# RustAudio/rodio

Measured on AMD Instinct MI355X. Metric: Msamples/s through resample+low_pass+mix pipeline, higher is better.
Workload: dtype f32; 1 GPU; 256 f32 stereo sources/GPU x 1048576 frames, 44.1->48 kHz linear resample + low_pass(200) + ordered Mixer sum, span_len=None; numpy default_rng(1234+s) U(-1,1)/256; in_frames=1048576, out_frames=1141308, channels=2, kernel=k_rlm_chunk

## Files before the change

rodio_amd/csrc/rh_pipeline.hip:

```cpp
#include "rh_pipeline_dev.h"

namespace {


__device__ __forceinline__ uint32_t rag_find_pairs(const Params &p, const uint32_t m_tile0, const uint32_t m_stable, const int lane, lds_u8 *lds, const uint32_t list_off);
template <int R, int KV, int C>
__device__ __forceinline__ void rag_run_pairs(const Params &p, unsigned long long *const rows, const uint32_t tile, const uint32_t n_pairs, const int lane, lds_u8 *lds, const uint32_t lds0,
                                              const uint32_t list_off, const uint32_t i_base, const uint32_t nvec, const uint32_t (&goff)[KV], const int (&offA)[R + 2], const float (&wgt)[R + 2],
                                              const float (&lM)[4], const float (&b15)[4], const float (&b31)[4], const float (&kM)[4], typename Chan<C>::V (&acc)[R]);

template <int R, int KV, int NS, bool FILT, bool RAG = false, int C = 2, bool SUMF = false>
__global__ __launch_bounds__(64, (R <= 4 ? (KV <= 5 ? 5 : 4) : R <= 6 ? 3 : R <= 12 ? 2 : 1)) void k_rlm_fast(const Params p) {
    typedef Chan<C> CH;
    typedef typename CH::V V;
    constexpr uint32_t FB = CH::kFB, VF = CH::kVF;
    static_assert(R <= kMaxR, "frames per lane");
    static_assert(NS >= 2 && NS <= 4, "ring depth");
    static_assert(KV * (NS - 1) < 64, "vmcnt range");
    constexpr uint32_t kStage = KV * 1024;
    extern __shared__ __attribute__((aligned(16))) unsigned char smem[];
    lds_u8 *const lds = (lds_u8 *)smem;
    const uint32_t lds0 = (uint32_t)(uintptr_t)lds;

    const int lane = threadIdx.x;
// ... 1124 lines not shown
            for (int u = 0; u < U; ++u) {
                const v4f v = __builtin_nontemporal_load(ptr + base + (uint64_t)u * 256u);
                acc[u].x = fma_(g, v.x, acc[u].x);
                acc[u].y = fma_(g, v.y, acc[u].y);
                acc[u].z = fma_(g, v.z, acc[u].z);
                acc[u].w = fma_(g, v.w, acc[u].w);
            }
        }
#pragma unroll
        for (int u = 0; u < U; ++u) *reinterpret_cast<v4f *>(y + 4 * (base + (uint64_t)u * 256u)) = acc[u];
    } else {
        for (int u = 0; u < U; ++u) {
            const uint64_t i = base + (uint64_t)u * 256u;
            if (i >= nvec) break;
            v4f a = v4f{0.f, 0.f, 0.f, 0.f};
            for (uint32_t s = 0; s < n_sources; ++s) {
                glb_cf4 *const ptr = (glb_cf4 *)(uintptr_t)(desc[4 * (uint64_t)s] + src_off);
                const float g = dgain[8 * (uint64_t)s + 4];
                const v4f v = ptr[i];
                a.x = fma_(g, v.x, a.x), a.y = fma_(g, v.y, a.y), a.z = fma_(g, v.z, a.z), a.w = fma_(g, v.w, a.w);
            }
            *reinterpret_cast<v4f *>(y + 4 * i) = a;
        }
    }
    if (blockIdx.x == 0) {
        const uint64_t t = nvec * 4 + threadIdx.x;
        if (t < n_floats) {
            float a = 0.f;
            for (uint32_t s = 0; s < n_sources; ++s) a = fma_(dgain[8 * (uint64_t)s + 4], ((glb_cf32 *)(uintptr_t)(desc[4 * (uint64_t)s] + src_off))[t], a);
            y[t] = a;
        }
        if (threadIdx.x == 0) {
            ydesc->data = desc_row;
            ydesc->frames = frames;
            ydesc->out_frames = out_frames;
            ydesc->gain = 1.0f;
            ydesc->pad[0] = ydesc->pad[1] = ydesc->pad[2] = 0;
        }
    }
}

template <int NS>
__global__ __launch_bounds__(64) void k_mix_ring(const SrcDesc *__restrict__ srcs, const uint32_t n_sources, float *__restrict__ y, const uint64_t n_floats, SrcDesc *__restrict__ ydesc,
                                                 const uint32_t frames, const uint32_t out_frames, const float *desc_row, const uint64_t src_off) {
    constexpr int KV = 8;
    constexpr uint32_t kStage = KV * 1024;
    __shared__ __attribute__((aligned(1024))) unsigned char smem[NS * kStage];
    lds_u8 *const lds = (lds_u8 *)smem;
    const uint32_t lds0 = (uint32_t)(uintptr_t)lds;
    typedef __attribute__((address_space(4))) const uint64_t cu64;
    typedef __attribute__((address_space(4))) const float cf32;
    cu64 *const desc = (cu64 *)(uintptr_t)srcs;
    cf32 *const dgain = (cf32 *)(uintptr_t)srcs;
    const int lane = threadIdx.x;
    const uint64_t nvec = n_floats / 4;
    const uint64_t v0 = (uint64_t)blockIdx.x * (KV * 64);
    uint32_t goff[KV];
#pragma unroll
    for (int k = 0; k < KV; ++k) {
        uint64_t j = v0 + (uint64_t)k * 64 + lane;
        j = j < nvec ? j : nvec - 1;
        goff[k] = (uint32_t)(j * 16);
    }
    auto stage_source = [&](uint32_t s_, uint32_t stage) {
        const void *data = (const void *)(uintptr_t)(desc[4 * (uint64_t)s_] + src_off);
#pragma unroll
        for (int k = 0; k < KV; ++k) glds16(data, goff[k], lds0 + stage * kStage + k * 1024);
    };
    v4f acc[KV];
#pragma unroll
    for (int k = 0; k < KV; ++k) acc[k] = v4f{0.f, 0.f, 0.f, 0.f};
    if (v0 < nvec) {
#pragma unroll
        for (int d = 0; d < NS - 1; ++d)
            if ((uint32_t)d < n_sources) stage_source(d, d);
        uint32_t st = 0;
        float g_next = n_sources ? dgain[4] : 0.f;
        for (uint32_t s_ = 0; s_ < n_sources; ++s_) {
            const float g = g_next;
            g_next = s_ + 1 < n_sources ? dgain[8 * (uint64_t)(s_ + 1) + 4] : 0.f;
            if (s_ + NS - 1 < n_sources) {
                uint32_t into = st + NS - 1;
                into = into >= (uint32_t)NS ? into - NS : into;
                stage_source(s_ + NS - 1, into);
                wait_vm<KV *(NS - 1)>();
            } else {
                const uint32_t left = n_sources - 1 - s_;
                wait_groups<KV, NS>((int)left);
            }
            const lds_u8 *buf = lds + st * kStage;
            v4f v[KV];
#pragma unroll
            for (int k = 0; k < KV; ++k) v[k] = *(const lds_f4 *)(buf + k * 1024 + lane * 16);
            asm volatile("s_waitcnt lgkmcnt(0)" ::: "memory");
#pragma unroll
            for (int k = 0; k < KV; ++k) {
                acc[k].x = fma_(g, v[k].x, acc[k].x);
                acc[k].y = fma_(g, v[k].y, acc[k].y);
                acc[k].z = fma_(g, v[k].z, acc[k].z);
                acc[k].w = fma_(g, v[k].w, acc[k].w);
            }
            st = st + 1 == (uint32_t)NS ? 0 : st + 1;
        }
        wait_vm<0>();
#pragma unroll
        for (int k = 0; k < KV; ++k) {
            const uint64_t j = v0 + (uint64_t)k * 64 + lane;
            if (j < nvec) *reinterpret_cast<v4f *>(y + 4 * j) = acc[k];
        }
    }
    if (blockIdx.x == 0) {
        const uint64_t t = nvec * 4 + lane;
        if (t < n_floats) {
            float a = 0.f;
            for (uint32_t s_ = 0; s_ < n_sources; ++s_) a = fma_(dgain[8 * (uint64_t)s_ + 4], ((glb_cf32 *)(uintptr_t)(desc[4 * (uint64_t)s_] + src_off))[t], a);
            y[t] = a;
        }
        if (lane == 0) {
            ydesc->data = desc_row;
            ydesc->frames = frames;
            ydesc->out_frames = out_frames;
            ydesc->gain = 1.0f;
            ydesc->pad[0] = ydesc->pad[1] = ydesc->pad[2] = 0;
        }
    }
}

struct ChunkArgs {
    const uint32_t *m_lo;
    unsigned long long *halo;
    const float *lookT;
    const float *powM;
    const float *uni;
};
constexpr uint32_t kChunkMultiMax = 7;
struct ChunkMulti {
    struct Entry {
        Params p;
        ChunkArgs q;
    };
    uint32_t n;
    uint32_t first[kChunkMultiMax + 1];
    float *sum_out;
    Entry e[kChunkMultiMax];
};
static_assert(sizeof(ChunkMulti) <= 4096, "the kernarg segment");
#if defined(RH_CHUNK_DIAG) && RH_CHUNK_DIAG == 3
#define RH_CPH(i) { const unsigned long long cph_now = __builtin_readcyclecounter(); if (lane == 0) atomicAdd(p.ticket + 8 + (i), (uint32_t)(cph_now - cph_last)); cph_last = cph_now; }
#define RH_CPH_DECL unsigned long long cph_last = __builtin_readcyclecounter();
#else
#define RH_CPH(i)
#define RH_CPH_DECL
#endif
template <int R, int C, int KV>
__device__ __forceinline__ void rlm_chunk_tile(const Params &p, const ChunkArgs &q, const uint32_t block) {
    typedef Chan<C> CH;
    typedef typename CH::V V;
    constexpr int NS = 2, H = 4;
    constexpr uint32_t FB = CH::kFB;
    constexpr uint32_t kStage = KV * 1024, P = kStage / FB;
    constexpr uint32_t MB = NS * kStage + 64;
    __shared__ __attribute__((aligned(1024))) unsigned char smem[MB + kStage + 64];
    lds_u8 *const lds = (lds_u8 *)smem;
    const uint32_t lds0 = (uint32_t)(uintptr_t)lds;
    typedef __attribute__((address_space(4))) const uint64_t cu64;
    typedef __attribute__((address_space(4))) const float cf32;
    typedef __attribute__((address_space(4))) const uint32_t cu32;
    cu64 *const desc = (cu64 *)(uintptr_t)p.srcs;
    cf32 *const dgain = (cf32 *)(uintptr_t)p.srcs;
    const int lane = threadIdx.x;
    uint32_t tile = block;
    if (!p.direct) {
        const uint32_t x = block & 7u;
        const uint32_t k = __builtin_amdgcn_readfirstlane(lane == 0 ? atomicAdd(p.ticket + 32u * (1u + x), 1u) - p.shard_base : 0u);
        tile = x + 8u * k;
        if (tile >= p.n_tiles) return;
    }
#ifdef RH_CHUNK_RAGSIM
    const uint32_t Ns = p.eq_frames;
    const uint32_t S = 2u * tile < p.n_tiles ? p.n_sources : (uint32_t)(((uint64_t)p.n_sources * 2u * (p.n_tiles - tile)) / p.n_tiles);
#else
    const uint32_t Ns = p.eq_frames, S = p.n_sources;
#endif
    const uint32_t m_lo = ((cu32 *)(uintptr_t)q.m_lo)[tile], m_hi = ((cu32 *)(uintptr_t)q.m_lo)[tile + 1];
    const uint32_t m0 = m_lo + (uint32_t)lane * R;
    int nfl;
    uint32_t n_t_v;
    float pwv[4];
    {
        const uint32_t n_t = m_hi - m_lo;
        nfl = (int)n_t - lane * R < 0 ? 0 : ((int)n_t - lane * R > R ? R : (int)n_t - lane * R);
        const uint32_t nl0 = (n_t + R - 1) / R;
        const uint32_t v = nl0 ? n_t - (nl0 - 1) * R : 0;
        n_t_v = n_t;
        asm volatile("v_mov_b32 %0, %1" : "=v"(n_t_v) : "s"(n_t));
        const float *pw = q.powM + 4 * v;
#pragma unroll
        for (int k = 0; k < 4; ++k) {
            pwv[k] = pw[k];
            asm volatile("" : "+v"(pwv[k]));
        }
    }
    const bool first = (m0 == 0);

    const uint32_t nvec = Ns * C / 4;
    const uint32_t v0 = tile * (KV * 64);
    uint32_t goff[KV];
#pragma unroll
    for (int k = 0; k < KV; ++k) {
        uint32_t j = v0 + (uint32_t)k * 64 + lane;
        j = j < nvec ? j : nvec - 1;
        goff[k] = j * 16;
    }
    const bool lin = v0 + (uint32_t)(KV * 64) <= nvec;
    auto stage_source = [&](uint32_t s_, uint32_t stage) {
        const void *data = (const void *)(uintptr_t)desc[4 * (uint64_t)s_];
        if (lin) {
            glds16_run<KV>(data, goff[0], lds0 + stage * kStage);
        } else {
#pragma unroll
            for (int k = 0; k < KV; ++k) glds16(data, goff[k], lds0 + stage * kStage + k * 1024);
        }
    };
    if (S) stage_source(0, 0);
    if (S > 1) stage_source(1, 1);
    const Tables *__restrict__ tb = p.tabs;
    float lM[4], b15[4], b31[4], kM[4];
    constexpr int NHV = H * FB / 16;
    const uint32_t Jc = p.J < tile ? p.J : tile;
    int want_look = (uint32_t)lane < Jc ? 1 : 0;
    uint64_t a_halo_pub = (uint64_t)(uintptr_t)(q.halo + (uint64_t)tile * 8 + (uint32_t)(lane >= 64 - NHV ? lane - (64 - NHV) : 0) * 4);
    uint64_t a_halo_poll = (uint64_t)(uintptr_t)(q.halo + (uint64_t)(tile ? tile - 1 : 0) * 8 + (lane < H * C ? lane : 0));
    uint64_t a_gran_pub = (uint64_t)(uintptr_t)(p.gran + (uint64_t)tile * 4 + (lane < 2 * C ? lane : 0));
    uint64_t a_gran_poll = (uint64_t)(uintptr_t)(p.gran + (uint64_t)(tile ? tile - 1 - (want_look ? lane : 0) : 0) * 4);
    uint64_t a_out = (uint64_t)(uintptr_t)(p.out + ((uint64_t)m_lo + (uint32_t)lane) * C);
    uint32_t epoch_v = p.epoch;
    float U = q.uni[lane < 61 ? lane : 60];
    asm volatile("" : "+v"(want_look), "+v"(a_halo_pub), "+v"(a_halo_poll), "+v"(a_gran_pub), "+v"(a_gran_poll), "+v"(a_out), "+v"(epoch_v), "+v"(U));
    {
        const uint32_t Jc0 = Jc;
        const float *kp = q.lookT + ((uint64_t)tile * p.J + ((uint32_t)lane < Jc0 ? lane : 0)) * 4;
#pragma unroll
        for (int k = 0; k < 4; ++k) {
            lM[k] = tb->laneM[lane][k];
            b15[k] = tb->bc15M[lane][k];
            b31[k] = tb->bc31M[lane][k];
            kM[k] = kp[k];
        }
    }
    int offA[R + 2];
    float wgt[R + 2];
    {
        const int64_t fbase = (int64_t)tile * P;
        Cursor c = cursor_at(first ? 0 : m0 - 2, p);
#pragma unroll
        for (int rr = 0; rr < R + 2; ++rr) {
#if defined(RH_CHUNK_DIAG) && RH_CHUNK_DIAG == 2
            offA[rr] = (int)MB + rr * 8;
            wgt[rr] = 0.5f;
            continue;
#endif
            const bool dummy = first && rr < 2;
            uint64_t i;
            uint32_t num;
            cursor_resolve(c, p, i, num);
            if (i + 1 >= Ns) {
                i = Ns - 1;
                num = 0;
            }
            int64_t f = (int64_t)i - fbase;
            f = f < -H ? -H : (f > (int64_t)P - 1 ? (int64_t)P - 1 : f);
            offA[rr] = dummy ? (int)MB : (int)MB + (int)f * (int)FB;
            wgt[rr] = dummy ? 0.0f : (float)num / p.Tf;
            if (!dummy) cursor_next(c, p);
        }
    }
    v4f acc[KV];
#pragma unroll
    for (int k = 0; k < KV; ++k) acc[k] = v4f{0.f, 0.f, 0.f, 0.f};
    {
        uint32_t st = 0;
        float g_next = S ? dgain[4] : 0.f;
        for (uint32_t s_ = 0; s_ < S; ++s_) {
            const float g = g_next;
            g_next = s_ + 1 < S ? dgain[8 * (uint64_t)(s_ + 1) + 4] : 0.f;
            if (s_ + 1 < S) wait_vm<KV>();
            else wait_vm<0>();
            const lds_u8 *buf = lds + st * kStage;
            v4f v[KV];
#pragma unroll
            for (int k = 0; k < KV; ++k) v[k] = *(const lds_f4 *)(buf + k * 1024 + lane * 16);
            asm volatile("s_waitcnt lgkmcnt(0)" ::: "memory");
            if (s_ + 2 < S) stage_source(s_ + 2, st);
#pragma unroll
            for (int k = 0; k < KV; ++k) {
                acc[k].x = fma_(g, v[k].x, acc[k].x);
                acc[k].y = fma_(g, v[k].y, acc[k].y);
                acc[k].z = fma_(g, v[k].z, acc[k].z);
                acc[k].w = fma_(g, v[k].w, acc[k].w);
            }
            st ^= 1u;
        }
    }
    RH_CPH_DECL
#if defined(RH_CHUNK_DIAG) && RH_CHUNK_DIAG < 3
    {
        float t = 0.f;
#pragma unroll
        for (int k = 0; k < KV; ++k) t += acc[k].x + acc[k].y + acc[k].z + acc[k].w;
#pragma unroll
        for (int rr = 0; rr < R + 2; ++rr) t += wgt[rr] + (float)offA[rr];
        p.out[(uint64_t)tile * 64 + lane] = t + lM[0] + b15[0] + b31[0] + kM[0] + (float)nfl + (first ? 1.f : 0.f);
        return;
    }
#endif
    if (lane >= 64 - NHV) {
        unsigned long long *hp = (unsigned long long *)(uintptr_t)a_halo_pub;
        const float e[4] = {acc[KV - 1].x, acc[KV - 1].y, acc[KV - 1].z, acc[KV - 1].w};
#pragma unroll
        for (int w = 0; w < 4; ++w) __hip_atomic_store(hp + w, ((unsigned long long)epoch_v << 32) | __float_as_uint(e[w]), __ATOMIC_RELAXED, __HIP_MEMORY_SCOPE_AGENT);
    }
#pragma unroll
    for (int k = 0; k < KV; ++k) *(lds_f4 *)(lds + MB + (uint32_t)(k * 64 + lane) * 16) = acc[k];
    if (lane == 0) *(lds_f4 *)(lds + MB + kStage) = v4f{0.f, 0.f, 0.f, 0.f};
    bool dead = false;
    if (tile == 0) {
        if (lane < H * C) *(RH_LDS float *)(lds + MB - H * FB + lane * 4) = 0.0f;
    } else {
        const bool want = lane < H * C;
        const unsigned long long *hp = (const unsigned long long *)(uintptr_t)a_halo_poll;
        unsigned long long hv = 0;
        bool ok = false;
        uint32_t spins = 0;
        while (true) {
            if (want && !ok) {
                hv = __hip_atomic_load(hp, __ATOMIC_RELAXED, __HIP_MEMORY_SCOPE_AGENT);
                ok = (uint32_t)(hv >> 32) == epoch_v;
            }
            if (__all(ok || !want)) break;
            if (++spins > kSpinLimit) {
                if (lane == 0) atomicOr(p.status, 1u);
                dead = true;
                break;
            }
            __builtin_amdgcn_s_sleep(1);
        }
        if (want) *(RH_LDS float *)(lds + MB - H * FB + lane * 4) = dead ? __builtin_nanf("") : __uint_as_float((uint32_t)hv);
    }
    asm volatile("s_waitcnt lgkmcnt(0)" ::: "memory");
    __builtin_amdgcn_wave_barrier();
    RH_CPH(0)

    const float b0 = readlane_f(U, 0), c1 = readlane_f(U, 1), c2 = readlane_f(U, 2), na1 = -readlane_f(U, 3), na2 = -readlane_f(U, 4);
    V out[R];
    V E1 = CH::zero(), E2 = CH::zero();
    {
        V ta[R + 2], tb2[R + 2];
#pragma unroll
        for (int rr = 0; rr < R + 2; ++rr) {
            ta[rr] = CH::ld_lds(lds + offA[rr]);
            tb2[rr] = CH::ld_lds(lds + offA[rr] + FB);
        }
        auto tap = [&](int rr) -> V {
            V x;
#pragma unroll
            for (int ch = 0; ch < C; ++ch) CH::set(x, ch, fma_(CH::get(tb2[rr], ch) - CH::get(ta[rr], ch), wgt[rr], CH::get(ta[rr], ch)));
            return x;
        };
        V x2 = first ? CH::zero() : tap(0);
        V x1 = first ? CH::zero() : tap(1);
        V w1 = CH::zero(), w2 = CH::zero();
#pragma unroll
        for (int r = 0; r < R; ++r) {
            const V x = tap(r + 2);
            V w;
#pragma unroll
            for (int ch = 0; ch < C; ++ch) {
                const float wc = fma_(na1, CH::get(w1, ch), fma_(na2, CH::get(w2, ch), fma_(c2, CH::get(x2, ch), c1 * CH::get(x1, ch))));
                CH::set(w, ch, wc);
                CH::set(out[r], ch, fma_(b0, CH::get(x, ch), wc));
            }
            w2 = w1;
            w1 = w;
            x2 = x1;
            x1 = x;
            E1 = vsel(r + 1 == nfl, w1, E1);
            E2 = vsel(r + 1 == nfl, w2, E2);
        }
    }
    RH_CPH(1)
    float Pq[2 * C];
#pragma unroll
    for (int k = 0; k < 2 * C; ++k) Pq[k] = 0.f;
    {
        const float Tm[4] = {readlane_f(U, 5), readlane_f(U, 6), readlane_f(U, 7), readlane_f(U, 8)};
#pragma unroll
        for (int ch = 0; ch < C; ++ch) mat_acc(Tm, CH::get(E1, ch), CH::get(E2, ch), Pq[2 * ch], Pq[2 * ch + 1]);
    }
    float own[2 * C];
#pragma unroll
    for (int k = 0; k < 2 * C; ++k) own[k] = Pq[k];
#define RH_CSCAN(K, N)                                                                             \
    {                                                                                              \
        float sq[2 * C];                                                                           \
        _Pragma("unroll") for (int k = 0; k < 2 * C; ++k) sq[k] = dpp0<kDppRowShr + N, 0xf>(Pq[k]); \
        const float sM[4] = {readlane_f(U, 9 + 4 * K), readlane_f(U, 10 + 4 * K), readlane_f(U, 11 + 4 * K), readlane_f(U, 12 + 4 * K)}; \
        _Pragma("unroll") for (int ch = 0; ch < C; ++ch) mat_acc(sM, sq[2 * ch], sq[2 * ch + 1], Pq[2 * ch], Pq[2 * ch + 1]); \
    }
    RH_CSCAN(0, 1)
    RH_CSCAN(1, 2)
    RH_CSCAN(2, 4)
    RH_CSCAN(3, 8)
#undef RH_CSCAN
    {
        float sq[2 * C];
#pragma unroll
        for (int k = 0; k < 2 * C; ++k) sq[k] = dpp0<kDppBcast15, 0xa>(Pq[k]);
#pragma unroll
        for (int ch = 0; ch < C; ++ch) mat_acc(b15, sq[2 * ch], sq[2 * ch + 1], Pq[2 * ch], Pq[2 * ch + 1]);
    }
    {
        float sq[2 * C];
#pragma unroll
        for (int k = 0; k < 2 * C; ++k) sq[k] = dpp0<kDppBcast31, 0xc>(Pq[k]);
#pragma unroll
        for (int ch = 0; ch < C; ++ch) mat_acc(b31, sq[2 * ch], sq[2 * ch + 1], Pq[2 * ch], Pq[2 * ch + 1]);
    }
    {
        const uint32_t n_t = (uint32_t)__builtin_amdgcn_readfirstlane((int)n_t_v);
        const int nl = (int)((n_t + R - 1) / R);
        float A[2 * C];
#pragma unroll
        for (int k = 0; k < 2 * C; ++k) A[k] = 0.f;
        if (nl >= 1) {
#pragma unroll
            for (int k = 0; k < 2 * C; ++k) A[k] = __int_as_float(__builtin_amdgcn_readlane(__float_as_int(own[k]), nl - 1));
        }
        if (nl >= 2) {
            const float M[4] = {readfirstlane_f(pwv[0]), readfirstlane_f(pwv[1]), readfirstlane_f(pwv[2]), readfirstlane_f(pwv[3])};
            float xp[2 * C];
#pragma unroll
            for (int k = 0; k < 2 * C; ++k) xp[k] = __int_as_float(__builtin_amdgcn_readlane(__float_as_int(Pq[k]), nl - 2));
#pragma unroll
            for (int ch = 0; ch < C; ++ch) mat_acc(M, xp[2 * ch], xp[2 * ch + 1], A[2 * ch], A[2 * ch + 1]);
        }
        if (lane < 2 * C) {
            float ev = A[0];
#pragma unroll
            for (int k = 1; k < 2 * C; ++k) ev = lane == k ? A[k] : ev;
            __hip_atomic_store((unsigned long long *)(uintptr_t)a_gran_pub, ((unsigned long long)epoch_v << 32) | __float_as_uint(ev), __ATOMIC_RELAXED, __HIP_MEMORY_SCOPE_AGENT);
        }
    }
    float Q[2 * C];
#pragma unroll
    for (int k = 0; k < 2 * C; ++k) Q[k] = dpp0<kDppWaveShr1, 0xf>(Pq[k]);
    RH_CPH(2)
    float c[2 * C];
#pragma unroll
    for (int k = 0; k < 2 * C; ++k) c[k] = 0.f;
    if (tile > 0) {
        const bool want = want_look != 0;
        const unsigned long long *gp = (const unsigned long long *)(uintptr_t)a_gran_poll;
        unsigned long long gv[2 * C];
#pragma unroll
        for (int k = 0; k < 2 * C; ++k) gv[k] = 0;
        bool ok = false;
        uint32_t spins = 0;
        while (true) {
            if (want && !ok) {
                bool all = true;
#pragma unroll
                for (int k = 0; k < 2 * C; ++k) {
                    gv[k] = __hip_atomic_load(gp + k, __ATOMIC_RELAXED, __HIP_MEMORY_SCOPE_AGENT);
                    all = all && ((uint32_t)(gv[k] >> 32) == epoch_v);
                }
                ok = all;
            }
            if (__all(ok || !want)) break;
            if (++spins > kSpinLimit) {
                if (lane == 0) atomicOr(p.status, 1u);
                dead = true;
                break;
            }
            __builtin_amdgcn_s_sleep(4);
        }
        if (lane == 0 && spins) atomicAdd(p.status + 1, spins);
        if (want && ok && !dead) {
#pragma unroll
            for (int ch = 0; ch < C; ++ch) mat_acc(kM, __uint_as_float((uint32_t)gv[2 * ch]), __uint_as_float((uint32_t)gv[2 * ch + 1]), c[2 * ch], c[2 * ch + 1]);
        }
#pragma unroll
        for (int k = 0; k < 2 * C; ++k) {
            c[k] += dpp0<kDppRowShr + 1, 0xf>(c[k]);
            c[k] += dpp0<kDppRowShr + 2, 0xf>(c[k]);
            c[k] += dpp0<kDppRowShr + 4, 0xf>(c[k]);
            c[k] += dpp0<kDppRowShr + 8, 0xf>(c[k]);
            c[k] = readlane_f(c[k], 15) + readlane_f(c[k], 31);
        }
    }
    if (dead) {
#pragma unroll
        for (int k = 0; k < 2 * C; ++k) c[k] = __builtin_nanf("");
    }
    RH_CPH(3)
#pragma unroll
    for (int ch = 0; ch < C; ++ch) mat_acc(lM, c[2 * ch], c[2 * ch + 1], Q[2 * ch], Q[2 * ch + 1]);
    constexpr uint32_t kRow = (R + 1) * FB;
    {
        lds_u8 *row = lds + (uint32_t)lane * kRow;
#pragma unroll
        for (int r = 0; r < R; ++r) {
            V y;
#pragma unroll
            for (int ch = 0; ch < C; ++ch) CH::set(y, ch, fma_(readlane_f(U, 25 + 2 * r), Q[2 * ch], fma_(readlane_f(U, 26 + 2 * r), Q[2 * ch + 1], CH::get(out[r], ch))));
            if (C == 2) *(lds_f2 *)(row + r * FB) = v2f{CH::get(y, 0), CH::get(y, C - 1)};
            else *(RH_LDS float *)(row + r * FB) = CH::get(y, 0);
        }
    }
    asm volatile("s_waitcnt lgkmcnt(0)" ::: "memory");
    __builtin_amdgcn_wave_barrier();
    {
        const uint32_t n_t = (uint32_t)__builtin_amdgcn_readfirstlane((int)n_t_v);
        float *ot = (float *)(uintptr_t)a_out;
        for (uint32_t f0 = 0; f0 < n_t; f0 += 64) {
            const uint32_t f = f0 + (uint32_t)lane;
            if (f < n_t) {
                const lds_u8 *src2 = lds + (f / R) * kRow + (f % R) * FB;
                if (C == 2) {
                    const v2f a = *(const lds_f2 *)src2;
                    *reinterpret_cast<float2 *>(ot + (uint64_t)f0 * 2) = make_float2(a.x, a.y);
                } else {
                    ot[f0] = *(const RH_LDS float *)src2;
                }
            }
        }
    }
    RH_CPH(4)
}
template <int R, int C, int KV>
__global__ __launch_bounds__(64, 2) void k_rlm_chunk(const Params p, const ChunkArgs q) {
    rlm_chunk_tile<R, C, KV>(p, q, blockIdx.x);
}
template <int R, int C, int KV>
__global__ __launch_bounds__(64, 2) void k_rlm_chunk_multi(const ChunkMulti m) {
    uint32_t k = 0;
#pragma unroll
    for (uint32_t i = 1; i < kChunkMultiMax; ++i) k += (i < m.n && blockIdx.x >= m.first[i]) ? 1u : 0u;
    uint32_t b0 = 0;
#pragma unroll
    for (uint32_t i = 1; i < kChunkMultiMax; ++i) b0 = (i == k) ? m.first[i] : b0;
    k = __builtin_amdgcn_readfirstlane(k);
    typedef const __attribute__((address_space(4))) unsigned char *cbytes;
    cbytes e = (cbytes)__builtin_amdgcn_kernarg_segment_ptr() + offsetof(ChunkMulti, e) + (size_t)k * sizeof(ChunkMulti::Entry);
    Params p;
    ChunkArgs q;
    typedef const __attribute__((address_space(4))) uint32_t *cwords;
    static_assert(sizeof(Params) % 4 == 0 && sizeof(ChunkArgs) % 4 == 0 && offsetof(ChunkMulti::Entry, q) % 4 == 0, "copied word by word");
    {
        cwords wp = (cwords)(e + offsetof(ChunkMulti::Entry, p)), wq = (cwords)(e + offsetof(ChunkMulti::Entry, q));
        uint32_t *dp = reinterpret_cast<uint32_t *>(&p), *dq = reinterpret_cast<uint32_t *>(&q);
#pragma unroll
        for (uint32_t i = 0; i < sizeof(Params) / 4; ++i) dp[i] = wp[i];
#pragma unroll
        for (uint32_t i = 0; i < sizeof(ChunkArgs) / 4; ++i) dq[i] = wq[i];
    }
    rlm_chunk_tile<R, C, KV>(p, q, blockIdx.x - b0);
}

#if defined(RH_CLS_DIAG) && RH_CLS_DIAG == 9
__device__ unsigned long long g_cls_stamp[2048 * 8 * 8];
#define RH_CLS_STAMP(i) { if (lane == 0 && tile < 2048 && k < 8) g_cls_stamp[((uint64_t)tile * 8 + k) * 8 + (i)] = wall_clock64(); }
#else
#define RH_CLS_STAMP(i)
#endif
#define RH_PARG(T, e, f) (*(const __attribute__((address_space(4))) T *)((e) + offsetof(ChunkMulti::Entry, p) + offsetof(Params, f)))
#define RH_QARG(T, e, f) (*(const __attribute__((address_space(4))) T *)((e) + offsetof(ChunkMulti::Entry, q) + offsetof(ChunkArgs, f)))
template <int R, int C, int KV>
__global__ __launch_bounds__(128, 2) void k_rlm_chunk_classes(const ChunkMulti m) {
    typedef Chan<C> CH;
    typedef typename CH::V V;
    constexpr int NS = 2, H = 4;
    constexpr uint32_t FB = CH::kFB;
    constexpr uint32_t kStage = KV * 1024, P = kStage / FB;
    constexpr uint32_t kCtl = NS * kStage;
    constexpr uint32_t kImg = kStage + 128;
    constexpr uint32_t MB0 = kCtl + 64 + 64;
    __shared__ __attribute__((aligned(1024))) unsigned char smem[kCtl + 64 + 2 * kImg];
    lds_u8 *const lds = (lds_u8 *)smem;
    const uint32_t lds0 = (uint32_t)(uintptr_t)lds;
    typedef __attribute__((address_space(4))) const uint64_t cu64;
    typedef __attribute__((address_space(4))) const float cf32;
    typedef __attribute__((address_space(4))) const uint32_t cu32;
    typedef const __attribute__((address_space(4))) unsigned char *cbytes;
    const cbytes kseg = (cbytes)__builtin_amdgcn_kernarg_segment_ptr();
    const int wave = __builtin_amdgcn_readfirstlane((int)(threadIdx.x >> 6));
    const int lane = (int)(threadIdx.x & 63u);
    const uint32_t n_cls = m.n;
    const Params &p0 = m.e[0].p;
    const uint32_t tile = blockIdx.x;
    const uint32_t Ns = p0.eq_frames;
    auto entry = [&](uint32_t k) -> cbytes { return kseg + offsetof(ChunkMulti, e) + (size_t)k * sizeof(ChunkMulti::Entry); };
    auto ctl_read = [&](uint32_t which) -> uint32_t {
        uint32_t v;
        asm volatile("ds_read_b32 %0, %1\n\ts_waitcnt lgkmcnt(0)" : "=v"(v) : "v"(lds0 + kCtl + which * 4) : "memory");
        return (uint32_t)__builtin_amdgcn_readfirstlane((int)v);
    };
    auto ctl_write = [&](uint32_t which, uint32_t v) {
        asm volatile("s_waitcnt lgkmcnt(0)" ::: "memory");
        if (lane == 0) *(RH_LDS uint32_t *)(lds + kCtl + which * 4) = v;
        asm volatile("s_waitcnt lgkmcnt(0)" ::: "memory");
    };
    if (wave == 0) {
        if (lane < 2) *(RH_LDS uint32_t *)(lds + kCtl + lane * 4) = 0u;
    }
    asm volatile("s_waitcnt lgkmcnt(0)\n\ts_barrier" ::: "memory");
    if (wave == 0) {
        const uint32_t nvec = Ns * C / 4;
        const uint32_t v0 = tile * (KV * 64);
        uint32_t goff[KV];
#pragma unroll
        for (int k = 0; k < KV; ++k) {
            uint32_t j = v0 + (uint32_t)k * 64 + lane;
            j = j < nvec ? j : nvec - 1;
            goff[k] = j * 16;
        }
        const bool lin = v0 + (uint32_t)(KV * 64) <= nvec;
        auto stage_source = [&](cu64 *desc, uint32_t s_, uint32_t stage) {
            const void *data = (const void *)(uintptr_t)desc[4 * (uint64_t)s_];
            if (lin) {
                glds16_run<KV>(data, goff[0], lds0 + stage * kStage);
            } else {
#pragma unroll
                for (int k = 0; k < KV; ++k) glds16(data, goff[k], lds0 + stage * kStage + k * 1024);
            }
        };
        constexpr int NHV = H * FB / 16;
        __builtin_amdgcn_s_setprio(3);
        uint32_t kc = 0, sc = 0;
        cu64 *ndesc = (cu64 *)(uintptr_t)RH_PARG(uint64_t, entry(0), srcs);
        uint32_t nS = RH_PARG(uint32_t, entry(0), n_sources);
        uint32_t nstage = 0;
        auto request_next = [&]() {
            if (kc >= n_cls) return false;
            stage_source(ndesc, sc, nstage);
            nstage ^= 1u;
            if (++sc == nS) {
                sc = 0;
                if (++kc < n_cls) {
                    ndesc = (cu64 *)(uintptr_t)RH_PARG(uint64_t, entry(kc), srcs);
                    nS = RH_PARG(uint32_t, entry(kc), n_sources);
                }
            }
            return true;
        };
        uint32_t ahead = 0;
        if (request_next()) ++ahead;
        if (request_next()) ++ahead;
        uint32_t st = 0;
        for (uint32_t k = 0; k < n_cls; ++k) {
            const cbytes e = entry(k);
            cf32 *const dgain = (cf32 *)(uintptr_t)RH_PARG(uint64_t, e, srcs);
            const uint32_t S = RH_PARG(uint32_t, e, n_sources);
            v4f acc[KV];
#pragma unroll
            for (int i = 0; i < KV; ++i) acc[i] = v4f{0.f, 0.f, 0.f, 0.f};
            float g_next = S ? dgain[4] : 0.f;
            for (uint32_t s_ = 0; s_ < S; ++s_) {
                const float g = g_next;
                g_next = s_ + 1 < S ? dgain[8 * (uint64_t)(s_ + 1) + 4] : 0.f;
                if (ahead > 1) wait_vm<KV>();
                else wait_vm<0>();
                --ahead;
                const lds_u8 *buf = lds + st * kStage;
                v4f v[KV];
#pragma unroll
                for (int i = 0; i < KV; ++i) v[i] = *(const lds_f4 *)(buf + i * 1024 + lane * 16);
                asm volatile("s_waitcnt lgkmcnt(0)" ::: "memory");
                if (request_next()) ++ahead;
#pragma unroll
                for (int i = 0; i < KV; ++i) {
                    acc[i].x = fma_(g, v[i].x, acc[i].x);
                    acc[i].y = fma_(g, v[i].y, acc[i].y);
                    acc[i].z = fma_(g, v[i].z, acc[i].z);
                    acc[i].w = fma_(g, v[i].w, acc[i].w);
                }
                st ^= 1u;
            }
            RH_CLS_STAMP(0)
            if (lane >= 64 - NHV) {
                unsigned long long *hp = (unsigned long long *)(uintptr_t)RH_QARG(uint64_t, e, halo) + (uint64_t)tile * 8 + (uint32_t)(lane - (64 - NHV)) * 4;
// ... 624 lines not shown

#define RH_FAST(r, kv, ns) Variant{r, kv, ns, &k_rlm_fast<r, kv, ns, true>, &k_rlm_fast<r, kv, ns, false>}
#define RH_WAVE(r, kv, ns) Variant{r, kv, ns, &k_rlm_wave<r, kv, ns, true>, &k_rlm_wave<r, kv, ns, false>}
const Variant kFast[] = {
#ifdef RH_DEV_VARIANTS
    RH_FAST(4, 2, 2), RH_FAST(4, 2, 3), RH_FAST(5, 3, 2), RH_FAST(6, 3, 2), RH_FAST(6, 3, 3), RH_FAST(8, 4, 2), RH_FAST(8, 4, 3), RH_FAST(9, 5, 2), RH_FAST(9, 5, 3), RH_FAST(12, 6, 3),
#else
    RH_FAST(3, 2, 2),   RH_FAST(3, 2, 3),   RH_FAST(3, 4, 2),  RH_FAST(3, 7, 2),
    RH_FAST(4, 2, 2),   RH_FAST(4, 2, 3),   RH_FAST(4, 3, 2),  RH_FAST(4, 3, 3),  RH_FAST(4, 5, 2),  RH_FAST(4, 9, 2),
    RH_FAST(5, 3, 2),   RH_FAST(5, 3, 3),   RH_FAST(5, 6, 2),
    RH_FAST(6, 3, 2),   RH_FAST(6, 3, 3),   RH_FAST(6, 4, 2),  RH_FAST(6, 4, 3),  RH_FAST(6, 7, 2),  RH_FAST(6, 14, 2),
    RH_FAST(7, 4, 2),   RH_FAST(7, 4, 3),   RH_FAST(7, 8, 2),
    RH_FAST(8, 4, 2),   RH_FAST(8, 4, 3),   RH_FAST(8, 4, 4),  RH_FAST(8, 5, 2),  RH_FAST(8, 5, 3),  RH_FAST(8, 9, 2),
    RH_FAST(9, 5, 2),   RH_FAST(9, 5, 3),   RH_FAST(9, 10, 2),
    RH_FAST(10, 5, 2),  RH_FAST(10, 5, 3),  RH_FAST(10, 6, 2), RH_FAST(10, 6, 3), RH_FAST(10, 11, 2),
    RH_FAST(12, 6, 2),  RH_FAST(12, 6, 3),  RH_FAST(12, 7, 2), RH_FAST(12, 7, 3), RH_FAST(12, 13, 2),
    RH_FAST(14, 7, 2),  RH_FAST(14, 8, 2),
    RH_FAST(16, 8, 2),  RH_FAST(16, 8, 3),  RH_FAST(16, 9, 2), RH_FAST(16, 9, 3),
    RH_FAST(18, 9, 2),  RH_FAST(18, 9, 3),  RH_FAST(18, 10, 2),
    RH_FAST(20, 10, 2), RH_FAST(20, 10, 3), RH_FAST(20, 11, 2),
#endif
};
const Variant kWave[] = {
    RH_WAVE(6, 3, 2), RH_WAVE(6, 4, 2), RH_WAVE(6, 7, 2), RH_WAVE(6, 14, 2), RH_WAVE(8, 4, 2), RH_WAVE(8, 4, 3), RH_WAVE(8, 5, 2), RH_WAVE(8, 9, 2),
    RH_WAVE(9, 5, 2), RH_WAVE(9, 5, 3), RH_WAVE(10, 5, 2), RH_WAVE(10, 5, 3), RH_WAVE(10, 6, 2), RH_WAVE(12, 6, 2), RH_WAVE(12, 6, 3), RH_WAVE(12, 7, 2),
};
#ifdef RH_RAG_NO_SUMF
#define RH_RAGN(r, kv, ns) Variant{r, kv, ns, &k_rlm_fast<r, kv, ns, true, true>, &k_rlm_resid<r, kv>}
#else
#define RH_RAGN(r, kv, ns) Variant{r, kv, ns, &k_rlm_fast<r, kv, ns, true, true, 2, true>, &k_rlm_resid<r, kv>}
#endif
#define RH_RAG(r, kv) RH_RAGN(r, kv, 2)
const Variant kRag[] = {
    RH_RAG(6, 3), RH_RAG(6, 4), RH_RAG(6, 7), RH_RAG(6, 14), RH_RAG(8, 4), RH_RAG(8, 5), RH_RAG(8, 9), RH_RAG(9, 5), RH_RAG(10, 5), RH_RAG(10, 6), RH_RAG(12, 6), RH_RAG(12, 7),
    RH_RAG(14, 7), RH_RAG(14, 8), RH_RAG(18, 9), RH_RAG(18, 10),
};
const Variant kRag1[] = {
#define RH_RAG1(r, kv) Variant{r, kv, 2, &k_rlm_fast<r, kv, 2, true, true, 1, true>, nullptr}
    RH_RAG1(6, 2), RH_RAG1(8, 2), RH_RAG1(8, 3), RH_RAG1(10, 3), RH_RAG1(12, 3), RH_RAG1(12, 4), RH_RAG1(16, 4), RH_RAG1(16, 5), RH_RAG1(18, 5),
#undef RH_RAG1
};
#define RH_FAST1(r, kv, ns) Variant{r, kv, ns, &k_rlm_fast<r, kv, ns, true, false, 1>, &k_rlm_fast<r, kv, ns, false, false, 1>}
#define RH_WAVE1(r, kv, ns) Variant{r, kv, ns, &k_rlm_wave<r, kv, ns, true, 1>, &k_rlm_wave<r, kv, ns, false, 1>}
const Variant kFast1[] = {
    RH_FAST1(4, 2, 2),  RH_FAST1(4, 3, 2),  RH_FAST1(4, 5, 2),  RH_FAST1(6, 2, 2),  RH_FAST1(6, 4, 2),  RH_FAST1(6, 7, 2),  RH_FAST1(8, 2, 2),   RH_FAST1(8, 3, 2),
    RH_FAST1(8, 5, 2),  RH_FAST1(8, 10, 2), RH_FAST1(9, 3, 2),  RH_FAST1(9, 5, 2),  RH_FAST1(10, 3, 2), RH_FAST1(10, 6, 2), RH_FAST1(12, 3, 2),  RH_FAST1(12, 4, 2),
    RH_FAST1(12, 7, 2), RH_FAST1(16, 4, 2), RH_FAST1(16, 5, 2), RH_FAST1(16, 9, 2), RH_FAST1(18, 5, 2), RH_FAST1(18, 5, 3), RH_FAST1(18, 10, 2), RH_FAST1(20, 5, 2),
    RH_FAST1(20, 6, 2), RH_FAST1(20, 11, 2),
};
const Variant kWave1[] = {
    RH_WAVE1(6, 2, 2), RH_WAVE1(6, 4, 2), RH_WAVE1(6, 7, 2), RH_WAVE1(8, 2, 2),  RH_WAVE1(8, 3, 2),  RH_WAVE1(8, 5, 2),  RH_WAVE1(8, 10, 2),
    RH_WAVE1(9, 3, 2), RH_WAVE1(9, 5, 2), RH_WAVE1(10, 3, 2), RH_WAVE1(10, 6, 2), RH_WAVE1(12, 3, 2), RH_WAVE1(12, 4, 2), RH_WAVE1(12, 7, 2),
};
#undef RH_FAST1
#undef RH_WAVE1
#undef RH_RAG
#undef RH_RAGN
#undef RH_FAST
#undef RH_WAVE
}

namespace rhp {

VariantTab variant_tab(TabKind kind, bool mono) {
    switch (kind) {
    case kTabFast: return mono ? tab_of(kFast1) : tab_of(kFast);
    case kTabWave: return mono ? tab_of(kWave1) : tab_of(kWave);
    default: return mono ? tab_of(kRag1) : tab_of(kRag);
    }
}

const void *chunk_kernel(int R, uint32_t channels, int KV) {
    if (channels == 2 && R == 9 && KV == 4) return reinterpret_cast<const void *>(&k_rlm_chunk<9, 2, 4>);
    if (channels == 2 && R == 18 && KV == 8) return reinterpret_cast<const void *>(&k_rlm_chunk<18, 2, 8>);
    if (channels == 2 && R == 18 && KV == 4) return reinterpret_cast<const void *>(&k_rlm_chunk<18, 2, 4>);
    if (channels == 1 && R == 18 && KV == 4) return reinterpret_cast<const void *>(&k_rlm_chunk<18, 1, 4>);
    if (channels == 1 && R == 18 && KV == 2) return reinterpret_cast<const void *>(&k_rlm_chunk<18, 1, 2>);
    return nullptr;
}

static const void *chunk_multi_kernel(int R, uint32_t channels, int KV) {
    if (channels == 2 && R == 9 && KV == 4) return reinterpret_cast<const void *>(&k_rlm_chunk_multi<9, 2, 4>);
    if (channels == 2 && R == 18 && KV == 8) return reinterpret_cast<const void *>(&k_rlm_chunk_multi<18, 2, 8>);
    if (channels == 2 && R == 18 && KV == 4) return reinterpret_cast<const void *>(&k_rlm_chunk_multi<18, 2, 4>);
    if (channels == 1 && R == 18 && KV == 4) return reinterpret_cast<const void *>(&k_rlm_chunk_multi<18, 1, 4>);
    if (channels == 1 && R == 18 && KV == 2) return reinterpret_cast<const void *>(&k_rlm_chunk_multi<18, 1, 2>);
    return nullptr;
}

static const void *chunk_classes_kernel(int R, uint32_t channels, int KV) {
    if (channels == 2 && R == 18 && KV == 8) return reinterpret_cast<const void *>(&k_rlm_chunk_classes<18, 2, 8>);
    if (channels == 2 && R == 18 && KV == 4) return reinterpret_cast<const void *>(&k_rlm_chunk_classes<18, 2, 4>);
    if (channels == 1 && R == 18 && KV == 4) return reinterpret_cast<const void *>(&k_rlm_chunk_classes<18, 1, 4>);
    if (channels == 1 && R == 18 && KV == 2) return reinterpret_cast<const void *>(&k_rlm_chunk_classes<18, 1, 2>);
    return nullptr;
}

rh_status chunk_launch_classes(rh_rlm *const *classes, float *const *rows, uint64_t row_capacity_frames, uint32_t n, float *dst_sum, rh_stream stream, bool *taken, bool *summed) {
    *taken = false;
    *summed = false;
    if (n < 2 || n > kChunkMultiMax || rh::knob(rh::K_CLASSES_ONE_BY_ONE)) return RH_OK;
    const void *fn = nullptr;
    for (uint32_t k = 0; k < n; ++k) {
        const rh_rlm *h = classes[k];
        if (!h || !h->cls.empty() || !h->plan || h->out_frames == 0 || row_capacity_frames < h->out_frames) return RH_OK;
        if (!h->chunk.ok || !mix_first_applies(h, *h->plan, h->n_sources, false, false)) return RH_OK;
        const void *f = chunk_multi_kernel(h->chunk.R, h->cfg.channels, h->chunk.KV);
        if (!f || (fn && f != fn)) return RH_OK;
        fn = f;
    }
    ChunkMulti m;
    memset(&m, 0, sizeof m);
    for (uint32_t k = 0; k < n; ++k) {
        rh_rlm *h = classes[k];
        h->collect = &m;
        const rh_status st = rlm_launch(h, 0, h->n_sources, rows[k], row_capacity_frames, nullptr, stream, 0, 0, StreamArgs{});
        h->collect = nullptr;
        if (st != RH_OK) return st;
        if (m.n != k + 1) return RH_ERR_UNSUPPORTED;
    }
    void *args[] = {&m};
    hipStream_t s = rh::as_stream(stream);
    const void *fn2 = rh::knob(rh::K_CLASSES_ONE_WAVE) ? nullptr : chunk_classes_kernel(classes[0]->chunk.R, classes[0]->cfg.channels, classes[0]->chunk.KV);
    bool same = fn2 != nullptr;
    for (uint32_t k = 0; k < n && same; ++k) {
        const rh_rlm *h = classes[k], *h0 = classes[0];
        same = h->exclusive && h->eq_frames == h0->eq_frames && h->out_frames == h0->out_frames && h->F == h0->F && h->T == h0->T && h->chunk_in == h0->chunk_in &&
               h->chunk_out == h0->chunk_out && h->chunk.n_tiles == h0->chunk.n_tiles && h->chunk.R == h0->chunk.R && h->chunk.KV == h0->chunk.KV && h->n_sources >= 1;
    }
    if (same) {
        int per_cu = 0;
        same = hipOccupancyMaxActiveBlocksPerMultiprocessor(&per_cu, fn2, 128, 0) == hipSuccess && per_cu >= 1 &&
               (uint64_t)classes[0]->chunk.n_tiles <= (uint64_t)per_cu * (uint64_t)rh::g_num_cus;
    }
    hipError_t e;
    if (same) {
        m.sum_out = dst_sum;
        e = hipLaunchKernel(fn2, dim3(classes[0]->chunk.n_tiles), dim3(128), args, 0, s);
        *summed = e == hipSuccess;
    } else {
        e = hipLaunchKernel(fn, dim3(m.first[m.n]), dim3(64), args, 0, s);
        if (e == hipSuccess)
            for (uint32_t k = 0; k < n; ++k) classes[k]->shard_base += (m.first[k + 1] - m.first[k]) / 8u;
    }
    if (e != hipSuccess) {
        rh::set_hip_error(e, "k_rlm_chunk_multi / k_rlm_chunk_classes launch");
        return RH_ERR_HIP;
    }
    for (uint32_t k = 0; k < n; ++k) mark_launch(classes[k], s);
    *taken = true;
    return RH_OK;
}

#if defined(RH_CLS_DIAG) && RH_CLS_DIAG == 9
extern "C" int rh_debug_cls_stamps(unsigned long long *dst, size_t n) {
    return (int)hipMemcpyFromSymbol(dst, HIP_SYMBOL(g_cls_stamp), n * sizeof(unsigned long long), 0, hipMemcpyDeviceToHost);
}
#endif
void launch_state(hipStream_t s, unsigned long long *gran, const Tables *tabs, uint32_t n_sources, uint32_t cols, uint32_t last_col, uint32_t J, uint32_t epoch, uint32_t next_epoch) {
    hipLaunchKernelGGL(k_rlm_state, dim3((n_sources + 63) / 64), dim3(64), 0, s, gran, tabs, n_sources, cols, last_col, J, epoch, next_epoch);
}

void launch_state_sum(hipStream_t s, const unsigned long long *gran, const SrcDesc *srcs, uint32_t n_sources, uint32_t cols, uint32_t tag, float *w_out) {
    hipLaunchKernelGGL(k_rlm_state_sum, dim3(1), dim3(256), 0, s, gran, srcs, n_sources, cols, tag, w_out);
}

bool mix_first_applies(const rh_rlm *p, const Plan &pl, uint32_t count, bool per_source_states, bool batch) {
    return &pl == &p->fast && p->filt && p->mix_first_on && !per_source_states && !batch && count >= 2 && !rh::knob(rh::K_NO_MIX_FIRST);
}

rh_status rlm_launch(rh_rlm *p, uint32_t first, uint32_t count, float *dst, uint64_t out_capacity_frames, uint64_t *out_frames, rh_stream stream, uint32_t batch_streams, uint64_t out_stride,
                            const StreamArgs &sa) {
    RH_REQUIRE_INIT();
    if (!p) return RH_ERR_INVALID;
    if (!p->cls.empty()) return RH_ERR_UNSUPPORTED;
    if (first > p->n_sources || count > p->n_sources - first) return RH_ERR_INVALID;
    if (out_frames) *out_frames = p->out_frames;
    if (p->out_frames == 0) return RH_OK;
    if (!dst || (reinterpret_cast<uintptr_t>(dst) & 15u)) return RH_ERR_INVALID;
    if (out_capacity_frames < p->out_frames) return RH_ERR_CAPACITY;
    hipStream_t s = rh::as_stream(stream);
    {
        const rh_status w = pre_launch(p, s);
        if (w != RH_OK) return w;
    }
    const Plan &pl = *p->plan;
    {
        const rh_status w = next_epoch(p, s);
        if (w != RH_OK) return w;
    }
    Params k;
    k.srcs = p->d_srcs + first;
    k.tabs = pl.d_tabs;
    k.out = dst;
    k.gran = p->d_gran;
    k.ticket = p->d_ctl;
    k.status = p->d_ctl + 1;
    k.out_frames = p->out_frames;
    k.chunk_in = sa.mode ? p->st_chunk_in : p->chunk_in;
    k.chunk_out = sa.mode ? p->st_chunk_out : p->chunk_out;
    k.n_sources = count;
    k.n_tiles = p->n_tiles;
    k.F = p->F;
    k.T = p->T;
    k.qF = p->F / p->T;
    k.rF = p->F % p->T;
    k.Tf = (float)p->T;
    k.rcpT = rh::lerp_rcp(p->T);
    k.epoch = p->epoch;
    k.J = pl.J;
    k.ticket_base = p->ticket_base;
    k.direct = 0;
    k.rag_merge = k.rag_pairs_from = k.rag_pairs_to = 0;
    k.prof = p->d_prof;
    k.eq_frames = p->eq_frames;
    k.batch_streams = batch_streams;
    k.shards = (batch_streams >= 16 && batch_streams % 8 == 0 && !rh::knob(rh::K_NO_TICKET_SHARDS)) ? 8u : 1u;
    k.shard_base = p->shard_base;
    k.out_stride = out_stride;
    k.st_mode = sa.mode;
    k.st_active = sa.active;
    k.st_m0 = sa.m0;
    k.st_g0 = sa.g0;
    k.st_mfirst = sa.mode ? p->st_mfirst : 0;
    k.st_win = sa.win;
    k.st_wout = sa.wout;
    k.gran_cols = sa.gran_cols ? sa.gran_cols : p->n_tiles;
    k.col0 = sa.gran_cols ? 1u : 0u;
    k.u = pl.uni;
    void *args[] = {&k};
    const uint64_t grid = (uint64_t)p->n_tiles * (batch_streams ? batch_streams : 1);
    if (grid > 0x7fffffffull) return RH_ERR_UNSUPPORTED;
    if (&pl == &p->pair && !sa.mode && !batch_streams) {
        Params k1 = k;
        k1.gran = p->d_gran + (uint64_t)count * p->n_tiles * 4;
        k1.eq_frames = p->rag_frames;
        void *args1[] = {&k1};
#ifdef RH_RAG_NO_SUMF
        const bool merge = false;
#else
        const bool merge = !rh::knob(rh::K_RAG_TWO_KERNELS) || !pl.v->plain;
#endif
        k1.rag_merge = merge ? 1u : 0u;
        k1.rag_pairs_from = p->rag_pairs_from;
        k1.rag_pairs_to = p->rag_pairs_to;
        uint32_t lds1 = pl.lds_bytes + 128u;
        if (const char *w = rh::knob(rh::K_RAG_RESIDENT)) {
            const int want = atoi(w);
            if (want >= 2 && want < 8) lds1 = std::max(lds1, (kLdsGranules / (uint32_t)want) * kLdsGranule);
        }
        const uint32_t grid8 = ((uint32_t)grid + 7u) & ~7u;
        k1.shards = 8;
        k1.shard_base = p->shard_base;
        hipError_t e1 = hipLaunchKernel(reinterpret_cast<const void *>(pl.v->filt), dim3(grid8), dim3(64), args1, lds1, s);
        if (e1 == hipSuccess) p->shard_base += grid8 / 8u;
        if (e1 == hipSuccess && !merge) {
            k.ticket_base = p->ticket_base;
            e1 = hipLaunchKernel(reinterpret_cast<const void *>(pl.v->plain), dim3((uint32_t)grid), dim3(64), args, 2u * (uint32_t)pl.v->KV * 1024u + 128u , s);
            p->ticket_base += (uint32_t)grid;
        }
        if (e1 != hipSuccess) {
            rh::set_hip_error(e1, "ragged batch launch");
            return RH_ERR_HIP;
        }
        return mark_launch(p, s);
    }
    if (p->chunk.ok && !sa.mode && mix_first_applies(p, pl, count, false, batch_streams != 0) && count == p->n_sources && first == 0) {
        const ChunkPlan &c = p->chunk;
        k.tabs = c.d_tabs;
        k.gran = c.d_gran;
        k.n_tiles = c.n_tiles;
        k.J = c.J;
        k.u = c.uni;
        ChunkArgs ca;
        ca.m_lo = c.d_mlo;
        ca.halo = c.d_halo;
        ca.lookT = c.d_look;
        ca.powM = c.d_pow;
        ca.uni = c.d_uni;
        k.direct = (c.direct && p->exclusive) ? 1u : 0u;
        if (p->collect) {
            ChunkMulti &m = *static_cast<ChunkMulti *>(p->collect);
            if (m.n >= kChunkMultiMax) return RH_ERR_UNSUPPORTED;
            k.direct = 0;
            const uint32_t g8 = (c.n_tiles + 7u) & ~7u;
            m.e[m.n].p = k;
            m.e[m.n].q = ca;
            m.first[m.n + 1] = m.first[m.n] + g8;
            m.n += 1;
            return RH_OK;
        }
        const uint32_t cgrid = k.direct ? c.n_tiles : (c.n_tiles + 7u) & ~7u;
        void *cargs[] = {&k, &ca};
        const hipError_t ce = hipLaunchKernel(c.fn, dim3(cgrid), dim3(64), cargs, 0, s);
        if (ce != hipSuccess) {
            rh::set_hip_error(ce, "k_rlm_chunk launch");
            return RH_ERR_HIP;
        }
        if (!k.direct) p->shard_base += cgrid / 8u;
        return mark_launch(p, s);
    }
    const bool pre = p->pre_filter;
    if (pre && (&pl != &p->fast || sa.mode || batch_streams)) return RH_ERR_UNSUPPORTED;
    if (pre || mix_first_applies(p, pl, count, sa.gran_cols != 0, batch_streams != 0)) {
        const uint64_t n_floats = (uint64_t)p->eq_frames * p->cfg.channels;
        const size_t row = (size_t)(((sa.mode ? (uint64_t)p->cfg.max_in_frames * p->cfg.channels : n_floats) + 3) & ~3ull);
// ... 54 lines not shown
```

Measured before the change: 1.676 million Msamples/s.

## Generalize chunk source ring depth, compact LDS overlay, add early halo polling

Parameterizes the chunk kernel's source staging ring to 2-4 stages with a peeled tail loop, and moves the output row staging into a region overlaid on the ring so LDS size becomes the max of ring and overlay. Optional knobs issue the halo/granule polls early, overlapping them with the last source loads, and hoist uniform and power-table loads behind the first stage issue. Poll loops now do their first load before entering the spin loop. The defaults keep a two-stage ring with early polling and hoisting off, so the main default effect is a smaller LDS footprint and restructured control flow.

```diff
diff --git a/rodio_amd/csrc/rh_pipeline.hip b/rodio_amd/csrc/rh_pipeline.hip
--- a/rodio_amd/csrc/rh_pipeline.hip
+++ b/rodio_amd/csrc/rh_pipeline.hip
@@ -1300,15 +1300,38 @@
 #define RH_CPH(i)
 #define RH_CPH_DECL
 #endif
+#if defined(RH_CHUNK_DIAG) && RH_CHUNK_DIAG == 9
+__device__ unsigned long long g_chunk_stamp[4096 * 4];
+#define RH_CHUNK_STAMP(i) { if (lane == 0 && tile < 4096) { g_chunk_stamp[(uint64_t)tile * 4 + (i)] = wall_clock64(); if ((i) == 0) g_chunk_stamp[(uint64_t)tile * 4 + 2] = ((unsigned long long)__builtin_amdgcn_s_getreg(20 | (31 << 11)) << 32) | __builtin_amdgcn_s_getreg(4 | (31 << 11)); } }
+#else
+#define RH_CHUNK_STAMP(i)
+#endif
+#ifndef RH_CHUNK_NS
+#define RH_CHUNK_NS 2
+#endif
+#ifndef RH_CHUNK_NS_MONO
+#define RH_CHUNK_NS_MONO RH_CHUNK_NS
+#endif
+#ifndef RH_CHUNK_EARLY
+#define RH_CHUNK_EARLY 0
+#endif
+#ifndef RH_CHUNK_HOIST
+#define RH_CHUNK_HOIST 0
+#endif
 template <int R, int C, int KV>
 __device__ __forceinline__ void rlm_chunk_tile(const Params &p, const ChunkArgs &q, const uint32_t block) {
     typedef Chan<C> CH;
     typedef typename CH::V V;
-    constexpr int NS = 2, H = 4;
+    constexpr int NS = C == 2 ? RH_CHUNK_NS : RH_CHUNK_NS_MONO, H = 4;
+    static_assert(NS >= 2 && NS <= 4, "wait_groups / the 6-bit vmcnt: rings of 2 .. 4 stages");
     constexpr uint32_t FB = CH::kFB;
     constexpr uint32_t kStage = KV * 1024, P = kStage / FB;
-    constexpr uint32_t MB = NS * kStage + 64;
-    __shared__ __attribute__((aligned(1024))) unsigned char smem[MB + kStage + 64];
+    constexpr uint32_t MB = 64;
+    constexpr uint32_t kRow = (R + 1) * FB, kRows = MB + kStage + 64;
+    constexpr uint32_t kRing = NS * kStage, kOver = kRows + 64 * kRow;
+    constexpr uint32_t kSmem = kRing > kOver ? kRing : kOver;
+    static_assert(kSmem <= 40960, "four workgroups per CU (160 KiB)");
+    __shared__ __attribute__((aligned(1024))) unsigned char smem[kSmem];
     lds_u8 *const lds = (lds_u8 *)smem;
     const uint32_t lds0 = (uint32_t)(uintptr_t)lds;
     typedef __attribute__((address_space(4))) const uint64_t cu64;
@@ -1335,6 +1358,10 @@
     int nfl;
     uint32_t n_t_v;
     float pwv[4];
+#if RH_CHUNK_HOIST
+    float U = q.uni[lane < 61 ? lane : 60];
+    uint32_t pw_v;
+#endif
     {
         const uint32_t n_t = m_hi - m_lo;
         nfl = (int)n_t - lane * R < 0 ? 0 : ((int)n_t - lane * R > R ? R : (int)n_t - lane * R);
@@ -1342,12 +1369,16 @@
         const uint32_t v = nl0 ? n_t - (nl0 - 1) * R : 0;
         n_t_v = n_t;
         asm volatile("v_mov_b32 %0, %1" : "=v"(n_t_v) : "s"(n_t));
+#if RH_CHUNK_HOIST
+        pw_v = v;
+#else
         const float *pw = q.powM + 4 * v;
 #pragma unroll
         for (int k = 0; k < 4; ++k) {
             pwv[k] = pw[k];
             asm volatile("" : "+v"(pwv[k]));
         }
+#endif
     }
     const bool first = (m0 == 0);
 
@@ -1370,8 +1401,25 @@
             for (int k = 0; k < KV; ++k) glds16(data, goff[k], lds0 + stage * kStage + k * 1024);
         }
     };
-    if (S) stage_source(0, 0);
-    if (S > 1) stage_source(1, 1);
+#if RH_CHUNK_HOIST
+    asm volatile("" : "+v"(U));
+#endif
+#pragma unroll
+    for (int i = 0; i < NS; ++i) {
+        if (S > (uint32_t)i) stage_source((uint32_t)i, (uint32_t)i);
+    }
+#if RH_CHUNK_HOIST
+    {
+        cu32 *pw = (cu32 *)(uintptr_t)(q.powM + 4 * pw_v);
+#pragma unroll
+        for (int k = 0; k < 4; ++k) {
+            const uint32_t w = pw[k];
+            uint32_t wv;
+            asm volatile("v_mov_b32 %0, %1" : "=v"(wv) : "s"(w));
+            pwv[k] = __uint_as_float(wv);
+        }
+    }
+#endif
     const Tables *__restrict__ tb = p.tabs;
     float lM[4], b15[4], b31[4], kM[4];
     constexpr int NHV = H * FB / 16;
@@ -1383,7 +1431,9 @@
     uint64_t a_gran_poll = (uint64_t)(uintptr_t)(p.gran + (uint64_t)(tile ? tile - 1 - (want_look ? lane : 0) : 0) * 4);
     uint64_t a_out = (uint64_t)(uintptr_t)(p.out + ((uint64_t)m_lo + (uint32_t)lane) * C);
     uint32_t epoch_v = p.epoch;
+#if !RH_CHUNK_HOIST
     float U = q.uni[lane < 61 ? lane : 60];
+#endif
     asm volatile("" : "+v"(want_look), "+v"(a_halo_pub), "+v"(a_halo_poll), "+v"(a_gran_pub), "+v"(a_gran_poll), "+v"(a_out), "+v"(epoch_v), "+v"(U));
     {
         const uint32_t Jc0 = Jc;
@@ -1426,20 +1476,23 @@
     v4f acc[KV];
 #pragma unroll
     for (int k = 0; k < KV; ++k) acc[k] = v4f{0.f, 0.f, 0.f, 0.f};
+    constexpr int E = RH_CHUNK_EARLY ? 1 + 2 * C : 0;
+    unsigned long long hv0 = 0, gv0[2 * C];
+#pragma unroll
+    for (int k = 0; k < 2 * C; ++k) gv0[k] = 0;
     {
         uint32_t st = 0;
         float g_next = S ? dgain[4] : 0.f;
-        for (uint32_t s_ = 0; s_ < S; ++s_) {
+        auto take = [&](const uint32_t s_, auto W, const bool refill) {
             const float g = g_next;
             g_next = s_ + 1 < S ? dgain[8 * (uint64_t)(s_ + 1) + 4] : 0.f;
-            if (s_ + 1 < S) wait_vm<KV>();
-            else wait_vm<0>();
+            wait_vm<decltype(W)::value>();
             const lds_u8 *buf = lds + st * kStage;
             v4f v[KV];
 #pragma unroll
             for (int k = 0; k < KV; ++k) v[k] = *(const lds_f4 *)(buf + k * 1024 + lane * 16);
             asm volatile("s_waitcnt lgkmcnt(0)" ::: "memory");
-            if (s_ + 2 < S) stage_source(s_ + 2, st);
+            if (refill) stage_source(s_ + NS, st);
 #pragma unroll
             for (int k = 0; k < KV; ++k) {
                 acc[k].x = fma_(g, v[k].x, acc[k].x);
@@ -1447,9 +1500,21 @@
                 acc[k].z = fma_(g, v[k].z, acc[k].z);
                 acc[k].w = fma_(g, v[k].w, acc[k].w);
             }
-            st ^= 1u;
-        }
-    }
+            st = st + 1 == (uint32_t)NS ? 0u : st + 1;
+        };
+        const uint32_t D = S < (uint32_t)NS ? S : (uint32_t)NS;
+        for (uint32_t s_ = 0; s_ < S - D; ++s_) take(s_, std::integral_constant<int, (NS - 1) * KV>(), true);
+        if (E) {
+            hv0 = __hip_atomic_load((RH_GLB unsigned long long *)(uintptr_t)a_halo_poll, __ATOMIC_RELAXED, __HIP_MEMORY_SCOPE_AGENT);
+#pragma unroll
+            for (int k = 0; k < 2 * C; ++k) gv0[k] = __hip_atomic_load((RH_GLB unsigned long long *)(uintptr_t)a_gran_poll + k, __ATOMIC_RELAXED, __HIP_MEMORY_SCOPE_AGENT);
+        }
+        if (NS > 3 && D > 3) take(S - 4, std::integral_constant<int, 3 * KV + E>(), false);
+        if (NS > 2 && D > 2) take(S - 3, std::integral_constant<int, 2 * KV + E>(), false);
+        if (D > 1) take(S - 2, std::integral_constant<int, KV + E>(), false);
+        if (D > 0) take(S - 1, std::integral_constant<int, 0>(), false);
+    }
+    RH_CHUNK_STAMP(0)
     RH_CPH_DECL
 #if defined(RH_CHUNK_DIAG) && RH_CHUNK_DIAG < 3
     {
@@ -1477,14 +1542,10 @@
     } else {
         const bool want = lane < H * C;
         const unsigned long long *hp = (const unsigned long long *)(uintptr_t)a_halo_poll;
-        unsigned long long hv = 0;
-        bool ok = false;
+        unsigned long long hv = E ? hv0 : __hip_atomic_load(hp, __ATOMIC_RELAXED, __HIP_MEMORY_SCOPE_AGENT);
+        bool ok = (uint32_t)(hv >> 32) == epoch_v;
         uint32_t spins = 0;
         while (true) {
-            if (want && !ok) {
-                hv = __hip_atomic_load(hp, __ATOMIC_RELAXED, __HIP_MEMORY_SCOPE_AGENT);
-                ok = (uint32_t)(hv >> 32) == epoch_v;
-            }
             if (__all(ok || !want)) break;
             if (++spins > kSpinLimit) {
                 if (lane == 0) atomicOr(p.status, 1u);
@@ -1492,6 +1553,10 @@
                 break;
             }
             __builtin_amdgcn_s_sleep(1);
+            if (want && !ok) {
+                hv = __hip_atomic_load(hp, __ATOMIC_RELAXED, __HIP_MEMORY_SCOPE_AGENT);
+                ok = (uint32_t)(hv >> 32) == epoch_v;
+            }
         }
         if (want) *(RH_LDS float *)(lds + MB - H * FB + lane * 4) = dead ? __builtin_nanf("") : __uint_as_float((uint32_t)hv);
     }
@@ -1610,20 +1675,14 @@
         const bool want = want_look != 0;
         const unsigned long long *gp = (const unsigned long long *)(uintptr_t)a_gran_poll;
         unsigned long long gv[2 * C];
-#pragma unroll
-        for (int k = 0; k < 2 * C; ++k) gv[k] = 0;
-        bool ok = false;
+        bool ok = true;
+#pragma unroll
+        for (int k = 0; k < 2 * C; ++k) {
+            gv[k] = E ? gv0[k] : __hip_atomic_load(gp + k, __ATOMIC_RELAXED, __HIP_MEMORY_SCOPE_AGENT);
+            ok = ok && ((uint32_t)(gv[k] >> 32) == epoch_v);
+        }
         uint32_t spins = 0;
         while (true) {
-            if (want && !ok) {
-                bool all = true;
-#pragma unroll
-                for (int k = 0; k < 2 * C; ++k) {
-                    gv[k] = __hip_atomic_load(gp + k, __ATOMIC_RELAXED, __HIP_MEMORY_SCOPE_AGENT);
-                    all = all && ((uint32_t)(gv[k] >> 32) == epoch_v);
-                }
-                ok = all;
-            }
             if (__all(ok || !want)) break;
             if (++spins > kSpinLimit) {
                 if (lane == 0) atomicOr(p.status, 1u);
@@ -1631,6 +1690,15 @@
                 break;
             }
             __builtin_amdgcn_s_sleep(4);
+            if (want && !ok) {
+                bool all = true;
+#pragma unroll
+                for (int k = 0; k < 2 * C; ++k) {
+                    gv[k] = __hip_atomic_load(gp + k, __ATOMIC_RELAXED, __HIP_MEMORY_SCOPE_AGENT);
+                    all = all && ((uint32_t)(gv[k] >> 32) == epoch_v);
+                }
+                ok = all;
+            }
         }
         if (lane == 0 && spins) atomicAdd(p.status + 1, spins);
         if (want && ok && !dead) {
@@ -1653,9 +1721,8 @@
     RH_CPH(3)
 #pragma unroll
     for (int ch = 0; ch < C; ++ch) mat_acc(lM, c[2 * ch], c[2 * ch + 1], Q[2 * ch], Q[2 * ch + 1]);
-    constexpr uint32_t kRow = (R + 1) * FB;
     {
-        lds_u8 *row = lds + (uint32_t)lane * kRow;
+        lds_u8 *row = lds + kRows + (uint32_t)lane * kRow;
 #pragma unroll
         for (int r = 0; r < R; ++r) {
             V y;
@@ -1673,7 +1740,7 @@
         for (uint32_t f0 = 0; f0 < n_t; f0 += 64) {
             const uint32_t f = f0 + (uint32_t)lane;
             if (f < n_t) {
-                const lds_u8 *src2 = lds + (f / R) * kRow + (f % R) * FB;
+                const lds_u8 *src2 = lds + kRows + (f / R) * kRow + (f % R) * FB;
                 if (C == 2) {
                     const v2f a = *(const lds_f2 *)src2;
                     *reinterpret_cast<float2 *>(ot + (uint64_t)f0 * 2) = make_float2(a.x, a.y);
@@ -1684,6 +1751,7 @@
         }
     }
     RH_CPH(4)
+    RH_CHUNK_STAMP(1)
 }
 template <int R, int C, int KV>
 __global__ __launch_bounds__(64, 2) void k_rlm_chunk(const Params p, const ChunkArgs q) {
@@ -2614,6 +2682,11 @@
     return RH_OK;
 }
 
+#if defined(RH_CHUNK_DIAG) && RH_CHUNK_DIAG == 9
+extern "C" int rh_debug_chunk_stamps(unsigned long long *dst, size_t n) {
+    return (int)hipMemcpyFromSymbol(dst, HIP_SYMBOL(g_chunk_stamp), n * sizeof(unsigned long long), 0, hipMemcpyDeviceToHost);
+}
+#endif
 #if defined(RH_CLS_DIAG) && RH_CLS_DIAG == 9
 extern "C" int rh_debug_cls_stamps(unsigned long long *dst, size_t n) {
     return (int)hipMemcpyFromSymbol(dst, HIP_SYMBOL(g_cls_stamp), n * sizeof(unsigned long long), 0, hipMemcpyDeviceToHost);
```

Measured after the change: 1.676 million Msamples/s. About the same (-0.0%).
